# ZenHKD/ocr-vi-invoice

Hardware: AMD Instinct MI355X
Metric: invoice images/sec end-to-end (det+rec) (higher is better)
Workload: dtype f16x2

## Files before the change

include/ocrvi.h:

```cpp
#ifndef OCRVI_H
#define OCRVI_H

#include <stddef.h>
#include <stdint.h>

#ifdef __cplusplus
extern "C" {
#endif

#define OCRVI_OK 0
#define OCRVI_EINVAL (-1)
#define OCRVI_EHIP (-2)
#define OCRVI_ENOMEM (-3)
#define OCRVI_EBLOB (-4)
#define OCRVI_ERANGE (-5)

typedef enum { OCRVI_F32 = 0, OCRVI_BF16 = 1, OCRVI_F16 = 2, OCRVI_F16X2 = 3 } ocrvi_dtype;

const char* ocrvi_last_error(void);
int ocrvi_abi_version(void);

typedef struct ocrvi_det ocrvi_det;

typedef struct {
// ... 205 lines not shown
int ocrvi_edit_distance(int device, const int32_t* pred_ids, int T, const int32_t* pred_lens, const int32_t* gt_ids, int G,
                        const int32_t* gt_lens, int B, int32_t* dist, void* stream);

int ocrvi_test_offset_conv(int device, int dtype, const float* x, const float* weight_host, const float* bias_host, int N, int C, int H, int W,
                           int stride, float* out, int iters, float* avg_ms);
int ocrvi_test_deform_conv(int device, int dtype, const float* x, const float* offset, const float* mask,
                           const float* weight_host, const float* bias_host, int N, int C, int H, int W, int Co,
                           int stride, int relu, float* out, int iters, float* avg_ms);
int ocrvi_test_deform_conv_res(int device, int dtype, const float* x, const float* offset, const float* mask,
                               const float* weight_host, const float* bias_host, const float* res, int N, int C, int H, int W, int Co,
                               int stride, int relu, float* out, int iters, float* avg_ms);
int ocrvi_test_deform_conv_raw(int device, int dtype, const float* x, const float* offset, const float* mask,
                               const float* weight_host, const float* bias_host, const float* res, int N, int C, int H, int W, int Co,
                               int stride, int relu, void* out_raw, float* out);
int ocrvi_test_dcn_plan(int dtype, int N, int C, int H, int W, int Co, int stride, int n_cu, int32_t plan[8]);
int ocrvi_test_conv(int device, int dtype, const float* x, const float* weight_host, const float* bias_host,
                    int N, int C, int H, int W, int Co, int ksize, int sh, int sw, int groups, int act, float* out,
                    int iters, float* avg_ms);
int ocrvi_test_conv_res(int device, int dtype, const float* x, const float* weight_host, const float* bias_host, const float* res, int N,
                        int C, int H, int W, int Co, int ksize, int res_mode, int act, float* out, int iters, float* avg_ms);
int ocrvi_test_bneck_tail(int device, const float* t1, const float* identity, const float* w2_host, const float* b2_host,
                          const float* w3_host, const float* b3_host, const float* w1_host, const float* b1_host, int N, int H, int W,
                          int no_phase_c, float* y_out, float* t1n_out, int iters, float* avg_ms);
int ocrvi_test_db_tail(int device, int dtype, const float* x, const float* dc1_w_bin_host, const float* dc1_b_bin_host,
                       const float* dc1_w_thr_host, const float* dc1_b_thr_host, const float* dc2_w_bin_host, const float* dc2_b_bin_host,
                       const float* dc2_w_thr_host, const float* dc2_b_thr_host, int N, int OH, int OW, int groups, int binary_only,
                       float* out, float* out2, int iters, float* avg_ms);
int ocrvi_test_gemm(int device, int dtype, const float* a, const float* weight_host, const float* bias_host, const float* res, int M,
                    int K, int N, int act, int res_post, int out_f32, float* out, int iters, float* avg_ms);
int ocrvi_test_gemm_raw(int device, int dtype, const float* a, const float* weight_host, const float* bias_host, const float* res, int M,
                        int K, int N, int act, int res_post, int out_f32, void* out_raw, float* out);
int ocrvi_test_ring_plan(int dtype, int amode, int M, int K, int N, int out_f32, int has_res, int n_cu, int32_t plan[8]);
int ocrvi_test_conv_raw(int device, int dtype, const float* x, const float* weight_host, const float* bias_host, const float* res, int N,
                        int C, int H, int W, int Co, int ksize, int sh, int sw, int groups, int act, int res_post, int out_f32, int in_place,
                        void* out_raw, float* out);
int ocrvi_test_gconv_plan(int dtype, int N, int C, int H, int W, int Co, int sh, int sw, int groups, int out_f32, int has_res, int n_cu,
                          int32_t plan[12]);
int ocrvi_test_stem_pool(int device, int dtype, const float* x, const float* weight_host, const float* bias_host, int N, int H, int W, int fused,
                         float* out, int iters, float* avg_ms);
int ocrvi_test_attention(int device, int dtype, const float* qkv, int B, int N, int heads, float* out, int iters,
                         float* avg_ms);

int ocrvi_test_mlp(int device, int dtype, float* x, const float* ln_g_host, const float* ln_b_host, const float* w1_host, const float* b1_host,
                   const float* w2_host, const float* b2_host, const float* next_g_host, const float* next_b_host, int want_xn, int M, int D,
                   float* xn_out, int iters, float* avg_ms);
int ocrvi_test_mlp_raw(int device, int dtype, float* x, const float* ln_g_host, const float* ln_b_host, const float* w1_host, const float* b1_host,
// ... 23 lines not shown
```

ocr_vi_invoice_amd/_lib.py:

```python
from __future__ import annotations

import ctypes as C
import os
from typing import Optional

_HERE = os.path.dirname(os.path.abspath(__file__))
LIB_PATH = os.environ.get("OCRVI_LIB") or os.path.join(_HERE, "lib", "libocrvi.so")

OCRVI_F32, OCRVI_BF16, OCRVI_F16, OCRVI_F16X2 = 0, 1, 2, 3
DTYPES = {"f32": OCRVI_F32, "fp32": OCRVI_F32, "float32": OCRVI_F32, "bf16": OCRVI_BF16, "bfloat16": OCRVI_BF16,
          "f16": OCRVI_F16, "fp16": OCRVI_F16, "float16": OCRVI_F16,
          "f16x2": OCRVI_F16X2}
ABI_VERSION = 5

EXPORTS = [
    "ocrvi_last_error", "ocrvi_abi_version",
    "ocrvi_det_create", "ocrvi_det_destroy", "ocrvi_det_workspace_bytes", "ocrvi_det_forward", "ocrvi_det_debug_features",
    "ocrvi_rec_create", "ocrvi_rec_destroy", "ocrvi_rec_workspace_bytes", "ocrvi_rec_forward", "ocrvi_rec_debug_features",
    "ocrvi_ctc_greedy", "ocrvi_normalize_u8", "ocrvi_resize_u8", "ocrvi_crop_resize_normalize", "ocrvi_db_postprocess", "ocrvi_db_boxes_batch",
    "ocrvi_unclip_polygon", "ocrvi_db_components_workspace_bytes", "ocrvi_db_components", "ocrvi_db_boxes_batch_sparse",
    "ocrvi_test_deform_conv", "ocrvi_test_offset_conv", "ocrvi_test_conv", "ocrvi_test_gemm", "ocrvi_test_attention", "ocrvi_test_mlp", "ocrvi_test_stem_pool", "ocrvi_test_pack_f16x2",
    "ocrvi_prof_enable", "ocrvi_prof_reset", "ocrvi_prof_report",
    "ocrvi_det_status", "ocrvi_rec_status", "ocrvi_range_reset", "ocrvi_range_flag",
    "ocrvi_resize_normalize_pages", "ocrvi_crop_resize_normalize_pages", "ocrvi_db_boxes_pages",
    "ocrvi_det_binary_workspace_bytes", "ocrvi_det_forward_binary",
    "ocrvi_four_point_transform", "ocrvi_warp_perspective_u8", "ocrvi_warp_perspective_pages",
    "ocrvi_test_layernorm", "ocrvi_test_frm_vertical", "ocrvi_test_asf", "ocrvi_test_maxpool", "ocrvi_test_db_maps", "ocrvi_test_ctc_logsoftmax",
    "ocrvi_det_eval_workspace_bytes", "ocrvi_det_eval", "ocrvi_ctc_loss", "ocrvi_edit_distance",
    "ocrvi_test_deform_conv_res",
    "ocrvi_enhance_init", "ocrvi_enhance_tables", "ocrvi_enhance_workspace_bytes", "ocrvi_enhance_u8",
    "ocrvi_rgb_to_lab_u8", "ocrvi_lab_to_rgb_u8", "ocrvi_clahe_lab_u8", "ocrvi_nlm_lab_u8", "ocrvi_sharpen_u8",
    "ocrvi_min_area_quads", "ocrvi_quad_crops", "ocrvi_crop_quad_resize_normalize_pages", "ocrvi_crop_quad_resize_normalize",
    "ocrvi_jpeg_info", "ocrvi_jpeg_parse", "ocrvi_jpeg_table_entry", "ocrvi_jpeg_decode_pages",
    "ocrvi_test_conv_res", "ocrvi_test_db_tail",
    "ocrvi_db_target_jobs", "ocrvi_db_target_maps", "ocrvi_resize_normalize_pad_pages",
    "ocrvi_test_mlp_raw",
    "ocrvi_test_bneck_tail",
    "ocrvi_jpeg_quant_tables", "ocrvi_jpeg_encode_header", "ocrvi_jpeg_encode_sizes", "ocrvi_jpeg_encode_table_entry", "ocrvi_jpeg_encode_pages",
    "ocrvi_test_gemm_raw", "ocrvi_test_ring_plan",
    "ocrvi_overlay_segments", "ocrvi_overlay_pages",
    "ocrvi_test_deform_conv_raw", "ocrvi_test_dcn_plan",
    "ocrvi_test_conv_raw", "ocrvi_test_gconv_plan",
    "ocrvi_png_info", "ocrvi_png_parse", "ocrvi_png_table_entry", "ocrvi_png_plan", "ocrvi_png_decode_pages",
]
PAGE_ENTRY = 4
DET_EVAL_RECORD_BYTES = 104
DET_EVAL_INT_SLOTS = ("tp", "fp", "fn", "positive_count", "negatives", "negative_count")
DET_EVAL_F64_SLOTS = ("pos_bce", "topk_bce", "dice_inter", "pred_mask", "gt_mask", "l1_num", "thresh_mask")
CTC_LOSS_MAX_TARGET = 1024
EDIT_DISTANCE_MAX_LEN = 2048
CLAHE_WORKSPACE_BYTES = 16384
ENHANCE_MIN_SIDE = 16
DB_TARGET_GT, DB_TARGET_MASK, DB_TARGET_THRESH = 0, 1, 2
DB_TARGET_JOB = 8
DB_TARGET_MAX_SIDE = 16384
JPEG_ENTRY = 64
PNG_ENTRY = 16
JPEG_ENC_ENTRY = 64
JPEG_HEADER_MAX = 640
OVERLAY_SEG = 8
OVERLAY_PRIM = 8
OVERLAY_MAX_COORD = 16384


class DetCfg(C.Structure):
    _fields_ = [("dtype", C.c_int32), ("k", C.c_float), ("max_batch", C.c_int32), ("backbone", C.c_int32), ("no_dcn", C.c_int32),
# ... 59 lines not shown
    lib.ocrvi_db_components_workspace_bytes.restype = sz
    lib.ocrvi_db_components.argtypes = [i32, vp, i32, i32, i32, C.c_float, vp, vp, vp, i32, vp, vp, C.c_longlong, vp, vp]
    lib.ocrvi_db_boxes_batch_sparse.argtypes = [vp, vp, vp, i32, vp, vp, C.c_longlong, i32, i32, i32, C.c_float, i32, C.c_float, C.c_float,
                                                C.c_double, C.c_double, i32, i32, i32, vp, vp, i32, vp, i32, vp]
    lib.ocrvi_unclip_polygon.argtypes = [vp, i32, C.c_double, vp, i32, C.POINTER(i32)]
    lib.ocrvi_db_boxes_batch.argtypes = [vp, i32, i32, i32, C.c_float, C.c_float, i32, C.c_float, C.c_float, C.c_double, C.c_double, i32, i32, i32,
                                         vp, vp, i32, vp, i32]
    lib.ocrvi_resize_normalize_pages.argtypes = [i32, vp, i32, i32, i32, f32p, vp]
    lib.ocrvi_crop_resize_normalize_pages.argtypes = [i32, vp, i32, i32p, i32, i32, i32, f32p, vp]
    lib.ocrvi_four_point_transform.argtypes = [vp, vp, vp, i32p, i32p]
    lib.ocrvi_warp_perspective_u8.argtypes = [i32, vp, i32, i32, vp, vp, i32, i32, vp]
    lib.ocrvi_warp_perspective_pages.argtypes = [i32, vp, vp, vp, i32, vp]
    lib.ocrvi_db_boxes_pages.argtypes = [vp, i32, i32, i32, C.c_float, C.c_float, i32, C.c_float, C.c_float, vp, vp, vp, vp, vp,
                                         vp, i32, vp, vp, vp, i32, vp, vp, i32]
    lib.ocrvi_test_deform_conv.argtypes = [i32, i32, f32p, f32p, f32p, vp, vp, i32, i32, i32, i32, i32, i32, i32, f32p, i32,
                                           C.POINTER(C.c_float)]
    lib.ocrvi_test_deform_conv_res.argtypes = [i32, i32, f32p, f32p, f32p, vp, vp, f32p, i32, i32, i32, i32, i32, i32, i32, f32p, i32,
                                               C.POINTER(C.c_float)]
    lib.ocrvi_test_offset_conv.argtypes = [i32, i32, f32p, vp, vp, i32, i32, i32, i32, i32, f32p, i32, C.POINTER(C.c_float)]
    lib.ocrvi_test_conv.argtypes = [i32, i32, f32p, vp, vp, i32, i32, i32, i32, i32, i32, i32, i32, i32, i32, f32p, i32,
                                    C.POINTER(C.c_float)]
    lib.ocrvi_test_conv_res.argtypes = [i32, i32, f32p, vp, vp, f32p, i32, i32, i32, i32, i32, i32, i32, i32, f32p, i32, C.POINTER(C.c_float)]
    lib.ocrvi_test_bneck_tail.argtypes = [i32, f32p, f32p, vp, vp, vp, vp, vp, vp, i32, i32, i32, i32, f32p, f32p, i32, C.POINTER(C.c_float)]
    lib.ocrvi_test_db_tail.argtypes = [i32, i32, f32p, vp, vp, vp, vp, vp, vp, vp, vp, i32, i32, i32, i32, i32, f32p, f32p, i32,
                                       C.POINTER(C.c_float)]
    lib.ocrvi_test_gemm.argtypes = [i32, i32, f32p, vp, vp, f32p, i32, i32, i32, i32, i32, i32, f32p, i32, C.POINTER(C.c_float)]
    lib.ocrvi_test_gemm_raw.argtypes = [i32, i32, f32p, vp, vp, f32p, i32, i32, i32, i32, i32, i32, vp, f32p]
    lib.ocrvi_test_ring_plan.argtypes = [i32, i32, i32, i32, i32, i32, i32, i32, C.POINTER(C.c_int32)]
    lib.ocrvi_test_deform_conv_raw.argtypes = [i32, i32, f32p, f32p, f32p, vp, vp, f32p, i32, i32, i32, i32, i32, i32, i32, vp, f32p]
    lib.ocrvi_test_dcn_plan.argtypes = [i32, i32, i32, i32, i32, i32, i32, i32, C.POINTER(C.c_int32)]
    lib.ocrvi_test_conv_raw.argtypes = [i32, i32, f32p, vp, vp, f32p] + [i32] * 13 + [vp, f32p]
    lib.ocrvi_test_gconv_plan.argtypes = [i32] * 12 + [C.POINTER(C.c_int32)]
    lib.ocrvi_test_stem_pool.argtypes = [i32, i32, f32p, vp, vp, i32, i32, i32, i32, f32p, i32, C.POINTER(C.c_float)]
    lib.ocrvi_test_attention.argtypes = [i32, i32, f32p, i32, i32, i32, f32p, i32, C.POINTER(C.c_float)]
    lib.ocrvi_test_mlp.argtypes = [i32, i32, f32p, vp, vp, vp, vp, vp, vp, vp, vp, i32, i32, i32, f32p, i32, C.POINTER(C.c_float)]
    lib.ocrvi_test_mlp_raw.argtypes = [i32, i32, f32p, vp, vp, vp, vp, vp, vp, vp, vp, i32, i32, vp, f32p, i32, C.POINTER(C.c_float)]
    lib.ocrvi_test_pack_f16x2.argtypes = [f32p, sz, vp, C.POINTER(C.c_float)]
    lib.ocrvi_test_layernorm.argtypes = [i32, i32, f32p, i32, i32, vp, vp, i32, i32, f32p]
    lib.ocrvi_test_frm_vertical.argtypes = [i32, i32, f32p, vp, i32, i32, i32, i32, f32p]
    lib.ocrvi_test_asf.argtypes = [i32, i32, f32p, f32p, f32p, f32p, vp, vp, i32, i32, i32, f32p]
    lib.ocrvi_test_maxpool.argtypes = [i32, i32, f32p, i32, i32, i32, i32, f32p]
    lib.ocrvi_test_db_maps.argtypes = [i32, f32p, f32p, C.c_float, f32p, f32p, f32p, sz]
    lib.ocrvi_test_ctc_logsoftmax.argtypes = [i32, f32p, i32, i32, i32, i32, f32p, i32p]
    lib.ocrvi_det_eval_workspace_bytes.argtypes = [i32, i32, i32, C.POINTER(sz)]
    lib.ocrvi_det_eval.argtypes = [i32, f32p, f32p, f32p, f32p, f32p, f32p, f32p, f32p, i32, i32, i32, C.c_double, vp, vp, sz, vp]
    lib.ocrvi_ctc_loss.argtypes = [i32, f32p, i32, i32, i32, i32p, i32, i32p, i32p, i32, vp, vp]
    lib.ocrvi_edit_distance.argtypes = [i32, i32p, i32, i32p, i32p, i32, i32p, i32, i32p, vp]
# ... 85 lines not shown
```

ocr_vi_invoice_amd/csrc/det_model.hip:

```cpp
#include <algorithm>
#include <memory>

#include "model.h"

using namespace ocrvi;

namespace {
const int kBlocks50[4] = {3, 4, 6, 3}, kBlocks18[4] = {2, 2, 2, 2};
const int kWidth[4] = {64, 128, 256, 512};
struct ResBlock {
    ConvLayer conv1, conv2, off, conv3, down;
    bool dcn = false, has_down = false;
    int stride = 1;
    void* tail_w = nullptr;
    float* tail_bias = nullptr;
    float tail_ws3 = 1.f, tail_ws1 = 1.f;
    bool tail = false, tail_c = false;
};
}

struct ocrvi_det {
    int device = 0;
    ocrvi_det_cfg cfg{};
    DeviceStore store;
    ConvLayer stem;
    std::vector<ResBlock> layers[4];
    ConvLayer lat[4], fpn[4];
    float *asf_w = nullptr, *asf_b = nullptr;
    ConvLayer head_conv, head_dc1;
    float* dc2_wb = nullptr;
    Tensor tap_c[4], tap_fused;
    bool basic = false;
    int expansion = 4;
    RangeWatch range;
};

extern "C" int ocrvi_det_create(int device, const void* blob_p, size_t blob_bytes, const ocrvi_det_cfg* cfg, ocrvi_det** out) {
    OCRVI_CHECK(cfg && out, OCRVI_EINVAL, "det_create: null argument");
    OCRVI_CHECK(dtype_valid(cfg->dtype), OCRVI_EINVAL, "det_create: bad dtype %d", cfg->dtype);
    OCRVI_CHECK(cfg->backbone == 0 || cfg->backbone == 1, OCRVI_EINVAL, "det_create: backbone %d (0 = ResNet-50, 1 = ResNet-18)", cfg->backbone);
// ... 38 lines not shown
            if (bk.dcn) OCRVI_TRY(load_conv(st, blob, p + ".conv2.off", 27, w, 3, 1, AM_CONV3, dt, true, &bk.off));
            if (!basic) OCRVI_TRY(load_conv(st, blob, p + ".conv3", 4 * w, w, 1, 1, AM_CONV1, dt, true, &bk.conv3));
            if (bk.has_down) OCRVI_TRY(load_conv(st, blob, p + ".down", ex * w, inpl, 1, 1, AM_CONV1, dt, true, &bk.down));
            inpl = ex * w;
        }
        for (int b = 0; b < nblk && !basic && dt == OCRVI_F16X2; ++b) {
            ResBlock& bk = h->layers[li][b];
            if (bk.dcn || bk.stride != 1 || !bk.conv2.quartets || w != 64 || bk.conv2.Np != 64 || bk.conv2.Cin_g != 64) continue;
            const std::string p = "layer" + std::to_string(li + 1) + "." + std::to_string(b);
            const std::string pn = "layer" + std::to_string(li + 1) + "." + std::to_string(b + 1);
            const BlobTensor *w3 = nullptr, *b3 = nullptr, *w1 = nullptr, *b1 = nullptr;
            OCRVI_TRY(blob.get(p + ".conv3.w", 256, 64, 1, 1, &w3));
            OCRVI_TRY(blob.get(p + ".conv3.b", 256, 0, 0, 0, &b3));
            if (b + 1 < nblk) {
                OCRVI_TRY(blob.get(pn + ".conv1.w", 64, 256, 1, 1, &w1));
                OCRVI_TRY(blob.get(pn + ".conv1.b", 64, 0, 0, 0, &b1));
            }
            PackedBneckTail pt = pack_bneck_tail(w3->data, b3->data, w1 ? w1->data : nullptr, b1 ? b1->data : nullptr);
            OCRVI_TRY(st.upload(pt.stream.data(), pt.stream.size(), &bk.tail_w));
            OCRVI_TRY(st.upload_f32(pt.bias, &bk.tail_bias));
            bk.tail_ws3 = pt.ws3; bk.tail_ws1 = pt.ws1;
            bk.tail = true; bk.tail_c = w1 != nullptr;
        }
    }
    for (int i = 0; i < 4; ++i) {
        OCRVI_TRY(load_conv(st, blob, "neck.lat" + std::to_string(i), 256, ex * kWidth[i], 1, 1, AM_CONV1, dt, true, &h->lat[i]));
        OCRVI_TRY(load_conv(st, blob, "neck.fpn" + std::to_string(i), 256, 256, 3, 1, AM_CONV3, dt, true, &h->fpn[i], nullptr, true));
    }
    {
        const BlobTensor *w = nullptr, *b = nullptr;
        OCRVI_TRY(blob.get("neck.asf.w", 4, 1024, 0, 0, &w));
        OCRVI_TRY(blob.get("neck.asf.b", 4, 0, 0, 0, &b));
        OCRVI_TRY(st.upload(w->data, 4096 * 4, (void**)&h->asf_w));
        OCRVI_TRY(st.upload(b->data, 16, (void**)&h->asf_b));
    }
    OCRVI_TRY(load_conv(st, blob, "head.conv", 128, 256, 3, 1, AM_CONV3, dt, true, &h->head_conv, nullptr, true));
    {
        std::vector<float> w2(2 * 64 * 4), b2(2);
        const char* names[2] = {"head.bin", "head.thr"};
        const float *dw[2] = {nullptr, nullptr}, *db[2] = {nullptr, nullptr};
        for (int br = 0; br < 2; ++br) {
            const BlobTensor *w = nullptr, *b = nullptr, *ww = nullptr, *bb = nullptr;
            OCRVI_TRY(blob.get(std::string(names[br]) + ".dc1.w", 64, 64, 2, 2, &w));
            OCRVI_TRY(blob.get(std::string(names[br]) + ".dc1.b", 64, 0, 0, 0, &b));
            dw[br] = w->data;
            db[br] = b->data;
// ... 89 lines not shown
    Tensor idn;
    OCRVI_TRY(identity(r, bk, x, y, &idn));
    ConvOpts o = conv_opts(1, 1, ACT_RELU);
    o.res = &idn; o.res_mode = RES_SAME;
    if (bk.dcn) OCRVI_TRY(dcn_offsets(r, bk, t1, y.h, y.w, 1, &o.offs));
    return conv(r, bk.conv2, t1, y, o);
}

static int fused_bottleneck(Runner& r, const ResBlock& bk, const Tensor& x, const Tensor& y, const Tensor& t1, bool have_t1,
                            const Tensor& t1_next) {
    if (!have_t1) OCRVI_TRY(conv(r, bk.conv1, x, t1, conv_opts(1, 0, ACT_RELU)));
    Tensor idn;
    OCRVI_TRY(identity(r, bk, x, y, &idn));
    OCRVI_CHECK(idn.c == 256 && y.c == 256 && t1.c == 64 && !idn.f32 && !y.f32, OCRVI_EINVAL, "det: fused layer1 chain on a foreign shape");
    if (r.dry()) return OCRVI_OK;
    BneckTailParams q;
    q.x = t1.p; q.w2 = bk.conv2.w; q.wt = bk.tail_w; q.bias2 = bk.conv2.bias; q.bias_t = bk.tail_bias;
    q.idn = idn.p; q.y = y.p; q.t1n = bk.tail_c ? t1_next.p : nullptr;
    q.n_img = x.n; q.H = y.h; q.W = y.w;
    q.ws2 = bk.conv2.wscale; q.ws3 = bk.tail_ws3; q.ws1 = bk.tail_ws1;
    return launch_bneck_tail(q, r.stream);
}

static int det_layer(const ocrvi_det& h, Runner& r, int li, Tensor* x) {
    const std::vector<ResBlock>& blocks = h.layers[li];
    Tensor cur = *x;
    const int N = cur.n, w = kWidth[li], cw = h.expansion * w, nb = (int)blocks.size();
    const int lh = cur.h / blocks[0].stride, lw = cur.w / blocks[0].stride;
    Tensor tap = r.alloc(N, lh, lw, cw);
    const size_t slot_mark = r.arena.mark();
    Tensor slot[2] = {r.alloc(N, lh, lw, cw), r.alloc(N, lh, lw, cw)};
    const bool fused_layer = !h.basic && blocks[0].tail;
    Tensor t1pp[2];
    if (fused_layer) { t1pp[0] = r.alloc(N, lh, lw, w); t1pp[1] = r.alloc(N, lh, lw, w); }
    bool have_t1 = false;
    for (int b = 0; b < nb; ++b) {
        const ResBlock& bk = blocks[b];
        Tensor y = b == nb - 1 ? tap : slot[b & 1];
        const size_t block_mark = r.arena.mark();
        if (fused_layer && bk.tail) {
            OCRVI_TRY(fused_bottleneck(r, bk, cur, y, t1pp[b & 1], have_t1, t1pp[(b + 1) & 1]));
            have_t1 = bk.tail_c;
        } else if (h.basic) {
            OCRVI_TRY(basic_block(r, bk, cur, y, w));
        } else {
            OCRVI_TRY(bottleneck(r, bk, cur, y, w));
        }
        r.arena.release(block_mark);
        cur = y;
    }
    r.arena.release(slot_mark);
    *x = cur;
    return OCRVI_OK;
}

static int det_neck(const ocrvi_det& h, Runner& r, const Tensor* feats, Tensor* fused) {
    const int N = feats[0].n;
    Tensor inner[4], p[4];
    for (int i = 3; i >= 0; --i) {
        inner[i] = r.alloc(N, feats[i].h, feats[i].w, 256);
        ConvOpts o;
        if (i < 3) { o.res = &inner[i + 1]; o.res_mode = RES_UP2; }
        OCRVI_TRY(conv(r, h.lat[i], feats[i], inner[i], o));
        p[i] = r.alloc(N, feats[i].h, feats[i].w, 256);
        OCRVI_TRY(conv(r, h.fpn[i], inner[i], p[i], conv_opts(1, 1, ACT_RELU)));
// ... 101 lines not shown
```

ocr_vi_invoice_amd/csrc/kernels.h:

```cpp
#pragma once
#include "common.h"

namespace ocrvi {

int k_nchw3_to_nhwc4_pad(int dtype, const float* x, void* y, int N, int H, int W, int pad_t, int pad_l, int Hp, int Wp, hipStream_t s);
int k_maxpool3x3s2(int dtype, const void* x, void* y, int N, int H, int W, int C, hipStream_t s);
bool stem_pool_eligible(int dtype, int cout, int Kp, int KH, int H, int W);
int k_stem_pool(int dtype, const void* xpad, const void* w, const float* bias, float wscale, void* y, int N, int H, int W, int Hp, int Wp,
                hipStream_t s);
int k_layernorm(int dtype, const void* x, int x_f32, void* out, int out_f32, const float* gamma, const float* beta, int rows, int D,
                hipStream_t s);
bool mlp_fused_eligible(int dtype, int D);
bool mlp_x2_eligible(int dtype, int D);
void pack_mlp_x2_stream(const float* w1, const float* w2, int D, std::vector<char>& out);
int k_mlp_x2(float* x, void* xn, const float* ln_g, const float* ln_b, const float* next_g, const float* next_b, const void* wstream, const float* b1,
             const float* b2, int M, int D, hipStream_t s);
void pack_mlp_stream(const float* w1, const float* w2, int D, int dtype, std::vector<char>& out);
int k_mlp_fused(int dtype, float* x, void* xn, const float* ln_g, const float* ln_b, const float* next_g, const float* next_b, const void* wstream,
                const float* b1, const float* b2, int M, int D, hipStream_t s);
int k_cast_from_f32(int dtype, const float* x, void* y, size_t n, hipStream_t s);
int k_nhwc_to_nchw_f32(int dtype, const void* x, float* y, int N, int H, int W, int C, int ld, int coff, hipStream_t s);

int k_attention(int dtype, const void* qkv, void* out, int B, int N, int heads, hipStream_t s, void* scratch = nullptr);
size_t attention_scratch_bytes(int dtype, int B, int N, int heads);
int k_frm_vertical(int dtype, const void* kv, const float* vq, void* out, int B, int H, int W, int D, hipStream_t s);

int k_asf(int dtype, const void* p2, const void* p3, const void* p4, const void* p5, const float* w, const float* b, float* scratch, void* out,
          int N, int H, int W, hipStream_t s);
size_t asf_scratch_bytes(int N, int H, int W);
int k_db_maps(const float* bin_logits, const float* thresh_logits, float k, float* binary, float* thresh, float* thresh_binary, size_t n,
              hipStream_t s);

int k_ctc_logsoftmax_argmax(const float* logits, int ld, float* log_probs, int32_t* argmax_ids, int B, int T, int C, hipStream_t s);
int k_ctc_argmax_tbc(const float* log_probs, int32_t* argmax_ids, int B, int T, int C, hipStream_t s);
int k_ctc_collapse(const int32_t* argmax_ids, int32_t* ids, int32_t* lens, int B, int T, int blank, hipStream_t s);

}
```

ocr_vi_invoice_amd/csrc/mlp_x2.hip:

```cpp
#include <stdlib.h>
#include <string.h>

#include "gemm_ring.h"
#include "kernels.h"

namespace ocrvi {
OCRVI_RANGE_FLAG_TU()

struct MlpX2Params {
    float* x = nullptr;
    void* xn = nullptr;
    const float* ln_g = nullptr;
    const float* ln_b = nullptr;
    const float* next_g = nullptr;
    const float* next_b = nullptr;
    const char* wstream = nullptr;
    const float* b1 = nullptr;
    const float* b2 = nullptr;
    int M = 0;
};

template <int D, int R, int TB, bool SPLIT>
__global__ __launch_bounds__(512 / TB, TB == 2 ? 1 : 2) void mlp_x2_kernel(const MlpX2Params p) {
    typedef f16x2_t T;
    typedef Mma<T>::u4v U;
    constexpr int NWV = 8 / TB, NT = 64 * NWV;
    constexpr int KS = D / 32;
    constexpr int NCH = 4 * D / 32;
    constexpr int NB2 = D / 16;
    constexpr int W1B = 32 * D * 4;
    constexpr int UNIT = SPLIT ? W1B : 2 * W1B;
    constexpr int IPW = UNIT / 1024 / NWV;
    constexpr int PF = R - 1;
    constexpr int NU = (NCH + 1) * (SPLIT ? 2 : 1);
    static_assert(UNIT % (1024 * NWV) == 0 && R >= 2, "ring geometry");
    extern __shared__ __attribute__((aligned(16))) char smem[];
    const unsigned lds0 = (unsigned)(size_t)(__attribute__((address_space(3))) char*)smem;
    float* const c_b1 = (float*)(smem + R * UNIT);
    float* const c_b2 = c_b1 + 4 * D;
    float* const c_g = c_b2 + D;
    float* const c_be = c_g + D;
    float* const c_ng = c_be + D;
    float* const c_nb = c_ng + D;

    const int tid = threadIdx.x, lane = tid & 63;
    const int wave = __builtin_amdgcn_readfirstlane(tid >> 6);
    const int lr = lane & 15, g = lane >> 4;
    const bool next_ln = p.next_g != nullptr;
    for (int i = tid; i < 4 * D; i += NT) c_b1[i] = p.b1[i];
    for (int i = tid; i < D; i += NT) {
        c_b2[i] = p.b2[i];
        c_g[i] = p.ln_g[i];
        c_be[i] = p.ln_b[i];
        c_ng[i] = next_ln ? p.next_g[i] : 1.f;
        c_nb[i] = next_ln ? p.next_b[i] : 0.f;
    }
    const float* const tail = (const float*)(p.wstream + (size_t)(NCH + 1) * 2 * W1B);
    const float ws1 = tail[0], ws2 = tail[1];
    __syncthreads();

    const int ntiles = (p.M + 127) >> 7;
    const int G = gridDim.x;
    const int my_tiles = (ntiles - (int)blockIdx.x + G - 1) / G;

    const char* const wbase = uniform_ptr(p.wstream);
    int prod_slot = 0, prod_mod = 0, cons_slot = 0;
    auto issue_unit = [&]() {
        const char* src = wbase + (size_t)prod_mod * UNIT + wave * 1024;
        const unsigned dst = lds0 + prod_slot * UNIT + wave * 1024;
#pragma unroll
        for (int j = 0; j < IPW; ++j) glds16(src + j * (NWV * 1024), (unsigned)lane * 16u, __builtin_amdgcn_readfirstlane(dst + j * (NWV * 1024)));
        prod_slot = prod_slot + 1 == R ? 0 : prod_slot + 1;
        prod_mod = prod_mod + 1 == NU ? 0 : prod_mod + 1;
    };
    auto next_unit = [&]() -> const char* {
        wait_vm_barrier<(PF - 1) * IPW>();
        issue_unit();
        const char* s = smem + cons_slot * UNIT;
        cons_slot = cons_slot + 1 == R ? 0 : cons_slot + 1;
        return s;
    };
    for (int i = 0; i < PF; ++i) issue_unit();
    const int sw = swz128(lr);
    const int fo0 = ((2 * g) ^ sw) << 4, fo1 = ((2 * g + 1) ^ sw) << 4;
    unsigned long long range_mask = 0;

    for (int t = 0; t < my_tiles; ++t) {
        const int tile = (int)blockIdx.x + t * G;
        const int tok0 = tile * 128 + wave * (16 * TB);
        U xH[KS][TB], xL[KS][TB];
#pragma unroll
        for (int b = 0; b < TB; ++b) {
            float xv[KS][8];
            const int tok = min(tok0 + 16 * b + lr, p.M - 1);
            const float* xr = p.x + (size_t)tok * D + 8 * g;
#pragma unroll
            for (int ks = 0; ks < KS; ++ks) {
                const float4 v0 = *(const float4*)(xr + 32 * ks), v1 = *(const float4*)(xr + 32 * ks + 4);
                xv[ks][0] = v0.x; xv[ks][1] = v0.y; xv[ks][2] = v0.z; xv[ks][3] = v0.w;
                xv[ks][4] = v1.x; xv[ks][5] = v1.y; xv[ks][6] = v1.z; xv[ks][7] = v1.w;
            }
            float sum = 0.f;
#pragma unroll
            for (int ks = 0; ks < KS; ++ks)
#pragma unroll
                for (int e = 0; e < 8; ++e) sum += xv[ks][e];
            sum += __shfl_xor(sum, 16);
            sum += __shfl_xor(sum, 32);
            const float mean = sum / (float)D;
            float sq = 0.f;
#pragma unroll
            for (int ks = 0; ks < KS; ++ks)
#pragma unroll
                for (int e = 0; e < 8; ++e) { const float d = xv[ks][e] - mean; sq += d * d; }
            sq += __shfl_xor(sq, 16);
            sq += __shfl_xor(sq, 32);
            const float rstd = rsqrtf(sq / (float)D + 1e-5f);
#pragma unroll
            for (int ks = 0; ks < KS; ++ks) {
                float o[8];
#pragma unroll
                for (int q = 0; q < 2; ++q) {
                    const float4 gv = *(const float4*)(c_g + 32 * ks + 8 * g + 4 * q), bv = *(const float4*)(c_be + 32 * ks + 8 * g + 4 * q);
                    o[4 * q] = (xv[ks][4 * q] - mean) * rstd * gv.x + bv.x;
                    o[4 * q + 1] = (xv[ks][4 * q + 1] - mean) * rstd * gv.y + bv.y;
                    o[4 * q + 2] = (xv[ks][4 * q + 2] - mean) * rstd * gv.z + bv.z;
                    o[4 * q + 3] = (xv[ks][4 * q + 3] - mean) * rstd * gv.w + bv.w;
                }
                const uint4 c0 = Chunk<T>::pack(o), c1 = Chunk<T>::pack(o + 4);
                Mma<T>::regroup(c0, c1, xH[ks][b], xL[ks][b]);
            }
        }
        wait_vm_only<0>();

        f32x4 acc2[NB2][TB];
#pragma unroll
        for (int a = 0; a < NB2; ++a)
#pragma unroll
            for (int b = 0; b < TB; ++b) acc2[a][b] = (f32x4){0.f, 0.f, 0.f, 0.f};

        f32x4 hacc[2][TB], hprev[2][TB];
        constexpr int NV = 8 * TB;
        auto gelu_vals = [&](int i0, int i1, const float* bp) {
#pragma unroll
            for (int i = i0; i < i1; ++i) {
                const int b = i >> 3, a = (i >> 2) & 1, r = i & 3;
                hprev[a][b][r] = gelu_erf(hprev[a][b][r] * ws1 + bp[16 * a + r]);
            }
        };
        auto g1 = [&](const char* U1, bool with_gelu, const float* bv) {
#pragma unroll
            for (int a = 0; a < 2; ++a)
#pragma unroll
                for (int b = 0; b < TB; ++b) hacc[a][b] = (f32x4){0.f, 0.f, 0.f, 0.f};
            constexpr int P1 = TB == 2 ? 1 : 2;
            uint4 wr[P1 + 1][2][2];
            auto rd1 = [&](int ks, int set) {
#pragma unroll
                for (int a = 0; a < 2; ++a) {
                    const char* r = U1 + (ks * 32 + 16 * a + lr) * 128;
                    wr[set][a][0] = *(const uint4*)(r + fo0);
                    wr[set][a][1] = *(const uint4*)(r + fo1);
                }
            };
#pragma unroll
            for (int i = 0; i < P1; ++i) rd1(i, i);
            __builtin_amdgcn_sched_barrier(0);
#pragma unroll
            for (int ks = 0; ks < KS; ++ks) {
                if (ks + P1 < KS) rd1(ks + P1, (ks + P1) % (P1 + 1));
                __builtin_amdgcn_sched_barrier(0);
#pragma unroll
                for (int a = 0; a < 2; ++a)
#pragma unroll
                    for (int b = 0; b < TB; ++b)
                        Mma<T>::three(Mma<T>::as_u4v(wr[ks % (P1 + 1)][a][0]), Mma<T>::as_u4v(wr[ks % (P1 + 1)][a][1]), xH[ks][b], xL[ks][b], hacc[a][b]);
                if (with_gelu) gelu_vals(NV * ks / KS, NV * (ks + 1) / KS, bv);
                __builtin_amdgcn_sched_barrier(0);
            }
        };
        auto g2 = [&](const char* U2) {
            constexpr int GB = 2 / TB, NG = NB2 / GB, PFG = 2;
            uint4 w2r[PFG + 1][GB][2];
            auto rd2 = [&](int grp, int set) {
#pragma unroll
                for (int i = 0; i < GB; ++i) {
                    const char* r = U2 + (16 * (grp * GB + i) + lr) * 128;
                    w2r[set][i][0] = *(const uint4*)(r + fo0);
                    w2r[set][i][1] = *(const uint4*)(r + fo1);
                }
            };
#pragma unroll
            for (int i = 0; i < PFG; ++i) rd2(i, i);
            U hH[TB], hL[TB];
#pragma unroll
            for (int b = 0; b < TB; ++b) {
                const float h0[4] = {hprev[0][b][0], hprev[0][b][1], hprev[0][b][2], hprev[0][b][3]};
                const float h1[4] = {hprev[1][b][0], hprev[1][b][1], hprev[1][b][2], hprev[1][b][3]};
                range_mask |= f16x2_out_of_range(h0) | f16x2_out_of_range(h1);
                const uint4 c0 = Chunk<T>::pack(h0), c1 = Chunk<T>::pack(h1);
                Mma<T>::regroup(c0, c1, hH[b], hL[b]);
            }
            __builtin_amdgcn_sched_barrier(0);
#pragma unroll
            for (int grp = 0; grp < NG; ++grp) {
                if (grp + PFG < NG) rd2(grp + PFG, (grp + PFG) % (PFG + 1));
                __builtin_amdgcn_sched_barrier(0);
#pragma unroll
                for (int i = 0; i < GB; ++i)
#pragma unroll
                    for (int b = 0; b < TB; ++b)
                        Mma<T>::three(Mma<T>::as_u4v(w2r[grp % (PFG + 1)][i][0]), Mma<T>::as_u4v(w2r[grp % (PFG + 1)][i][1]), hH[b], hL[b], acc2[grp * GB + i][b]);
                __builtin_amdgcn_sched_barrier(0);
            }
        };
        auto keep = [&]() {
#pragma unroll
            for (int a = 0; a < 2; ++a)
#pragma unroll
                for (int b = 0; b < TB; ++b) hprev[a][b] = hacc[a][b];
        };
        auto second = [&](const char* U1) -> const char* {
            if constexpr (SPLIT) {
                return next_unit();
            } else {
                return U1 + W1B;
            }
        };
        auto bias_of = [&](int c) {
            int l = threadIdx.x;
            asm volatile("" : "+v"(l));
            return c_b1 + 32 * c + 4 * ((l & 63) >> 4);
        };
        {
            const char* const U1 = next_unit();
            g1(U1, false, bias_of(0));
            (void)second(U1);
        }
        keep();
        for (int k = 1; k < NCH; ++k) {
            const char* const U1 = next_unit();
            g1(U1, true, bias_of(k - 1));
            g2(second(U1));
            keep();
        }
        {
            const char* const U1 = next_unit();
            gelu_vals(0, NV, bias_of(NCH - 1));
            g2(second(U1));
        }

        const int pn_tok = lane >> 2, pn_g = lane & 3;
        const int pn_src = 4 * (16 * pn_g + pn_tok);
#pragma unroll
        for (int b = 0; b < TB; ++b) {
#pragma unroll
            for (int a = 0; a < NB2; ++a)
#pragma unroll
                for (int r = 0; r < 4; ++r)
                    acc2[a][b][r] = __int_as_float(__builtin_amdgcn_ds_bpermute(pn_src, __float_as_int(acc2[a][b][r])));
            const int tok = tok0 + 16 * b + pn_tok;
            const bool ok = tok < p.M;
            float* xr = p.x + (size_t)(ok ? tok : 0) * D + 4 * pn_g;
            float sum = 0.f;
            float4 rvs[NB2];
#pragma unroll
            for (int a = 0; a < NB2; ++a) rvs[a] = *(const float4*)(xr + 16 * a);
#pragma unroll
            for (int a = 0; a < NB2; ++a) {
                const float4 bv2 = *(const float4*)(c_b2 + 16 * a + 4 * pn_g);
                const float4 rv = rvs[a];
                f32x4 v = acc2[a][b];
                v[0] = v[0] * ws2 + bv2.x + rv.x; v[1] = v[1] * ws2 + bv2.y + rv.y; v[2] = v[2] * ws2 + bv2.z + rv.z; v[3] = v[3] * ws2 + bv2.w + rv.w;
                acc2[a][b] = v;
                if (ok) *(float4*)(xr + 16 * a) = make_float4(v[0], v[1], v[2], v[3]);
                sum += v[0] + v[1] + v[2] + v[3];
            }
            if (p.xn) {
                float mean = 0.f, rstd = 1.f;
                if (next_ln) {
                    sum += __shfl_xor(sum, 1);
                    sum += __shfl_xor(sum, 2);
                    mean = sum / (float)D;
                    float sq = 0.f;
#pragma unroll
// ... 57 lines not shown
            }
        }
    }
    std::vector<char> chunks(buf.size() * 4);
    convert_to_dtype(buf.data(), buf.size(), OCRVI_F16X2, chunks.data());
    out.assign(chunks.size() + 8, 0);
    for (size_t r = 0; r < nrows; ++r) {
        const uint64_t* src = (const uint64_t*)(chunks.data() + r * 128);
        uint64_t q[16];
        for (int k = 0; k < 4; ++k) {
            q[4 * k] = src[4 * k]; q[4 * k + 1] = src[4 * k + 2]; q[4 * k + 2] = src[4 * k + 1]; q[4 * k + 3] = src[4 * k + 3];
        }
        const int row = rowidx[r], sw = ((row >> 1) & 1) | (((row >> 3) & 1) << 2);
        uint64_t* dst = (uint64_t*)(out.data() + r * 128);
        for (int ch = 0; ch < 8; ++ch) {
            dst[2 * (ch ^ sw)] = q[2 * ch];
            dst[2 * (ch ^ sw) + 1] = q[2 * ch + 1];
        }
    }
    const float tail[2] = {1.0f / s1, 1.0f / s2};
    memcpy(out.data() + chunks.size(), tail, 8);
}

template <int D, int R, int TB, bool SPLIT>
static int launch_mlp_x2(const MlpX2Params& p, hipStream_t s) {
    const int smem = R * (SPLIT ? 128 : 256) * D + 9 * D * 4;
    auto kern = mlp_x2_kernel<D, R, TB, SPLIT>;
    OCRVI_TRY(ensure_max_smem((const void*)kern, smem));
    int n_cu = 0;
    OCRVI_TRY(device_cus(&n_cu));
    const int ntiles = (p.M + 127) / 128;
    int grid = std::min(ntiles, n_cu);
    grid = cdiv(ntiles, cdiv(ntiles, grid));
    hipLaunchKernelGGL(kern, dim3(grid), dim3(512 / TB), smem, s, p);
    OCRVI_HIP(hipGetLastError());
    return OCRVI_OK;
}

int k_mlp_x2(float* x, void* xn, const float* ln_g, const float* ln_b, const float* next_g, const float* next_b, const void* wstream, const float* b1,
             const float* b2, int M, int D, hipStream_t s) {
    OCRVI_CHECK((D == 128 || D == 256 || D == 384) && x && ln_g && ln_b && wstream && b1 && b2 && M > 0 && M < (1 << 24), OCRVI_EINVAL,
                "mlp_x2: bad argument (D %d, M %d)", D, M);
    MlpX2Params p;
    p.x = x; p.xn = xn; p.ln_g = ln_g; p.ln_b = ln_b; p.next_g = next_g; p.next_b = next_b; p.wstream = (const char*)wstream; p.b1 = b1; p.b2 = b2; p.M = M;
    char tag[64];
    snprintf(tag, sizeof(tag), "mlp_fused_d%d_f16x2", D);
    ProfScope ps(tag, 2.0 * M * 8.0 * D * D, (double)M * D * (8.0 + (xn ? 4.0 : 0.0)) + 8.0 * D * D * 4.0, s);
    if (D == 128) return launch_mlp_x2<128, 4, 1, false>(p, s);
    if (D == 256) return launch_mlp_x2<256, 2, 1, false>(p, s);
    return launch_mlp_x2<384, 3, 2, true>(p, s);
}

}
```

Baseline: 323.4.

## Fuse bottleneck conv3 and next block's conv1 into one chained MLP-style kernel

Adds a bottleneck mode to the fused two-GEMM MLP kernel so a block's conv3 (plus identity residual and ReLU) and the next block's conv1 (ReLU) run in one kernel. The conv3 output is written to y while staying in registers to feed conv1, which saves a kernel launch and a global re-read of the 4w-channel activation. It applies to detector layers of width 128/256 when the f16x2 path is eligible. The added identity prefetch and vmcnt-based pipelining make the kernel more complex and raise register pressure.

Result: no change. 326.3, median of 6 (+0.9%).

```diff
diff --git a/include/ocrvi.h b/include/ocrvi.h
--- a/include/ocrvi.h
+++ b/include/ocrvi.h
@@ -251,6 +251,9 @@
 int ocrvi_test_bneck_tail(int device, const float* t1, const float* identity, const float* w2_host, const float* b2_host,
                           const float* w3_host, const float* b3_host, const float* w1_host, const float* b1_host, int N, int H, int W,
                           int no_phase_c, float* y_out, float* t1n_out, int iters, float* avg_ms);
+int ocrvi_test_bneck_chain(int device, const float* t2, const float* identity, const float* w3_host, const float* b3_host,
+                           const float* w1_host, const float* b1_host, int N, int P, int H, int W, int idn_c, int idn_c0, float* y_out,
+                           float* t1n_out, int iters, float* avg_ms);
 int ocrvi_test_db_tail(int device, int dtype, const float* x, const float* dc1_w_bin_host, const float* dc1_b_bin_host,
                        const float* dc1_w_thr_host, const float* dc1_b_thr_host, const float* dc2_w_bin_host, const float* dc2_b_bin_host,
                        const float* dc2_w_thr_host, const float* dc2_b_thr_host, int N, int OH, int OW, int groups, int binary_only,
diff --git a/ocr_vi_invoice_amd/_lib.py b/ocr_vi_invoice_amd/_lib.py
--- a/ocr_vi_invoice_amd/_lib.py
+++ b/ocr_vi_invoice_amd/_lib.py
@@ -42,6 +42,7 @@
     "ocrvi_test_deform_conv_raw", "ocrvi_test_dcn_plan",
     "ocrvi_test_conv_raw", "ocrvi_test_gconv_plan",
     "ocrvi_png_info", "ocrvi_png_parse", "ocrvi_png_table_entry", "ocrvi_png_plan", "ocrvi_png_decode_pages",
+    "ocrvi_test_bneck_chain",
 ]
 PAGE_ENTRY = 4
 DET_EVAL_RECORD_BYTES = 104
@@ -147,7 +148,8 @@
                                     C.POINTER(C.c_float)]
     lib.ocrvi_test_conv_res.argtypes = [i32, i32, f32p, vp, vp, f32p, i32, i32, i32, i32, i32, i32, i32, i32, f32p, i32, C.POINTER(C.c_float)]
     lib.ocrvi_test_bneck_tail.argtypes = [i32, f32p, f32p, vp, vp, vp, vp, vp, vp, i32, i32, i32, i32, f32p, f32p, i32, C.POINTER(C.c_float)]
-    lib.ocrvi_test_db_tail.argtypes = [i32, i32, f32p, vp, vp, vp, vp, vp, vp, vp, vp, i32, i32, i32, i32, i32, f32p, f32p, i32,
+    lib.ocrvi_test_bneck_chain.argtypes = [i32, f32p, f32p, vp, vp, vp, vp, i32, i32, i32, i32, i32, i32, f32p, f32p, i32, C.POINTER(C.c_float)]
+    lib.ocrvi_test_db_tail.argtypes =[i32, i32, f32p, vp, vp, vp, vp, vp, vp, vp, vp, i32, i32, i32, i32, i32, f32p, f32p, i32,
                                        C.POINTER(C.c_float)]
     lib.ocrvi_test_gemm.argtypes = [i32, i32, f32p, vp, vp, f32p, i32, i32, i32, i32, i32, i32, f32p, i32, C.POINTER(C.c_float)]
     lib.ocrvi_test_gemm_raw.argtypes = [i32, i32, f32p, vp, vp, f32p, i32, i32, i32, i32, i32, i32, vp, f32p]
diff --git a/ocr_vi_invoice_amd/csrc/det_model.hip b/ocr_vi_invoice_amd/csrc/det_model.hip
--- a/ocr_vi_invoice_amd/csrc/det_model.hip
+++ b/ocr_vi_invoice_amd/csrc/det_model.hip
@@ -16,6 +16,9 @@
     float* tail_bias = nullptr;
     float tail_ws3 = 1.f, tail_ws1 = 1.f;
     bool tail = false, tail_c = false;
+    void* chain_w = nullptr;
+    float *chain_b3 = nullptr, *chain_b1 = nullptr;
+    bool chain = false;
 };
 }
 
@@ -100,6 +103,22 @@
             bk.tail_ws3 = pt.ws3; bk.tail_ws1 = pt.ws1;
             bk.tail = true; bk.tail_c = w1 != nullptr;
         }
+        for (int b = 0; b + 1 < nblk && !basic && (w == 128 || w == 256) && mlp_x2_eligible(dt, w); ++b) {
+            ResBlock& bk = h->layers[li][b];
+            const std::string p = "layer" + std::to_string(li + 1) + "." + std::to_string(b);
+            const std::string pn = "layer" + std::to_string(li + 1) + "." + std::to_string(b + 1);
+            const BlobTensor *w3 = nullptr, *b3 = nullptr, *w1 = nullptr, *b1 = nullptr;
+            OCRVI_TRY(blob.get(p + ".conv3.w", 4 * w, w, 1, 1, &w3));
+            OCRVI_TRY(blob.get(p + ".conv3.b", 4 * w, 0, 0, 0, &b3));
+            OCRVI_TRY(blob.get(pn + ".conv1.w", w, 4 * w, 1, 1, &w1));
+            OCRVI_TRY(blob.get(pn + ".conv1.b", w, 0, 0, 0, &b1));
+            std::vector<char> stream;
+            pack_mlp_x2_stream(w3->data, w1->data, w, stream);
+            OCRVI_TRY(st.upload(stream.data(), stream.size(), &bk.chain_w));
+            OCRVI_TRY(st.upload(b3->data, (size_t)4 * w * 4, (void**)&bk.chain_b3));
+            OCRVI_TRY(st.upload(b1->data, (size_t)w * 4, (void**)&bk.chain_b1));
+            bk.chain = true;
+        }
     }
     for (int i = 0; i < 4; ++i) {
         OCRVI_TRY(load_conv(st, blob, "neck.lat" + std::to_string(i), 256, ex * kWidth[i], 1, 1, AM_CONV1, dt, true, &h->lat[i]));
@@ -235,6 +254,24 @@
     return launch_bneck_tail(q, r.stream);
 }
 
+static int chain_bottleneck(Runner& r, const ResBlock& bk, const Tensor& x, const Tensor& y, int w, const Tensor& t1_own, bool have_t1,
+                            const Tensor& t1_next) {
+    Tensor t1 = t1_own;
+    if (!have_t1) {
+        t1 = r.alloc(x.n, x.h, x.w, w);
+        OCRVI_TRY(conv(r, bk.conv1, x, t1, conv_opts(1, 0, ACT_RELU)));
+    }
+    Tensor t2 = r.alloc(x.n, y.h, y.w, w);
+    ConvOpts o2 = conv_opts(bk.stride, 1, ACT_RELU);
+    if (bk.dcn) OCRVI_TRY(dcn_offsets(r, bk, t1, y.h, y.w, bk.stride, &o2.offs));
+    OCRVI_TRY(conv(r, bk.conv2, t1, t2, o2));
+    Tensor idn;
+    OCRVI_TRY(identity(r, bk, x, y, &idn));
+    OCRVI_CHECK(idn.c == 4 * w && y.c == 4 * w && t1_next.c == w && !idn.f32 && !y.f32, OCRVI_EINVAL, "det: fused conv3 -> conv1 chain on a foreign shape");
+    if (r.dry()) return OCRVI_OK;
+    return k_bneck_chain(t2.p, idn.p, idn.c, bk.chain_w, bk.chain_b3, bk.chain_b1, y.p, t1_next.p, y.n * y.h * y.w, w, r.stream);
+}
+
 static int det_layer(const ocrvi_det& h, Runner& r, int li, Tensor* x) {
     const std::vector<ResBlock>& blocks = h.layers[li];
     Tensor cur = *x;
@@ -243,9 +280,9 @@
     Tensor tap = r.alloc(N, lh, lw, cw);
     const size_t slot_mark = r.arena.mark();
     Tensor slot[2] = {r.alloc(N, lh, lw, cw), r.alloc(N, lh, lw, cw)};
-    const bool fused_layer = !h.basic && blocks[0].tail;
+    const bool fused_layer = !h.basic && blocks[0].tail, chain_layer = !h.basic && blocks[0].chain;
     Tensor t1pp[2];
-    if (fused_layer) { t1pp[0] = r.alloc(N, lh, lw, w); t1pp[1] = r.alloc(N, lh, lw, w); }
+    if (fused_layer || chain_layer) { t1pp[0] = r.alloc(N, lh, lw, w); t1pp[1] = r.alloc(N, lh, lw, w); }
     bool have_t1 = false;
     for (int b = 0; b < nb; ++b) {
         const ResBlock& bk = blocks[b];
@@ -254,6 +291,19 @@
         if (fused_layer && bk.tail) {
             OCRVI_TRY(fused_bottleneck(r, bk, cur, y, t1pp[b & 1], have_t1, t1pp[(b + 1) & 1]));
             have_t1 = bk.tail_c;
+        } else if (chain_layer && (bk.chain || have_t1)) {
+            if (bk.chain) {
+                OCRVI_TRY(chain_bottleneck(r, bk, cur, y, w, t1pp[b & 1], have_t1, t1pp[(b + 1) & 1]));
+            } else {
+                Tensor t2 = r.alloc(N, lh, lw, w);
+                ConvOpts o2 = conv_opts(bk.stride, 1, ACT_RELU);
+                if (bk.dcn) OCRVI_TRY(dcn_offsets(r, bk, t1pp[b & 1], lh, lw, bk.stride, &o2.offs));
+                OCRVI_TRY(conv(r, bk.conv2, t1pp[b & 1], t2, o2));
+                ConvOpts o3 = conv_opts(1, 0, ACT_RELU);
+                o3.res = &cur; o3.res_mode = RES_SAME;
+                OCRVI_TRY(conv(r, bk.conv3, t2, y, o3));
+            }
+            have_t1 = bk.chain;
         } else if (h.basic) {
             OCRVI_TRY(basic_block(r, bk, cur, y, w));
         } else {
diff --git a/ocr_vi_invoice_amd/csrc/kernels.h b/ocr_vi_invoice_amd/csrc/kernels.h
--- a/ocr_vi_invoice_amd/csrc/kernels.h
+++ b/ocr_vi_invoice_amd/csrc/kernels.h
@@ -15,6 +15,8 @@
 void pack_mlp_x2_stream(const float* w1, const float* w2, int D, std::vector<char>& out);
 int k_mlp_x2(float* x, void* xn, const float* ln_g, const float* ln_b, const float* next_g, const float* next_b, const void* wstream, const float* b1,
              const float* b2, int M, int D, hipStream_t s);
+int k_bneck_chain(const void* t2, const void* idn, int ldr, const void* wstream, const float* b3, const float* b1, void* y, void* t1n, int M, int P,
+                  hipStream_t s);
 void pack_mlp_stream(const float* w1, const float* w2, int D, int dtype, std::vector<char>& out);
 int k_mlp_fused(int dtype, float* x, void* xn, const float* ln_g, const float* ln_b, const float* next_g, const float* next_b, const void* wstream,
                 const float* b1, const float* b2, int M, int D, hipStream_t s);
diff --git a/ocr_vi_invoice_amd/csrc/mlp_x2.hip b/ocr_vi_invoice_amd/csrc/mlp_x2.hip
--- a/ocr_vi_invoice_amd/csrc/mlp_x2.hip
+++ b/ocr_vi_invoice_amd/csrc/mlp_x2.hip
@@ -18,10 +18,27 @@
     const float* b1 = nullptr;
     const float* b2 = nullptr;
     int M = 0;
+    const void* t2 = nullptr;
+    const void* idn = nullptr;
+    void* y = nullptr;
+    void* t1n = nullptr;
+    void* dump_page = nullptr;
+    int ldr = 0;
 };
 
-template <int D, int R, int TB, bool SPLIT>
+template <int OFF> __device__ __forceinline__ void gload16so(u32x4& dst, const char* sbase, unsigned voff) {
+    asm volatile("global_load_dwordx4 %0, %1, %2 offset:%3" : "=v"(dst) : "v"(voff), "s"(sbase), "n"(OFF) : "memory");
+}
+__device__ __forceinline__ float f16x2_elem(const u32x4& u, int r) {
+    union { unsigned w; f16_t h[2]; } c;
+    c.w = r < 2 ? u.x : u.y;
+    const unsigned lw = r < 2 ? u.z : u.w;
+    return (r & 1) ? fma_mix_hi(1.0f, lw, (float)c.h[1]) : fma_mix_lo(1.0f, lw, (float)c.h[0]);
+}
+
+template <int D, int R, int TB, bool SPLIT, bool BN = false>
 __global__ __launch_bounds__(512 / TB, TB == 2 ? 1 : 2) void mlp_x2_kernel(const MlpX2Params p) {
+    static_assert(!BN || (TB == 1 && !SPLIT), "bottleneck mode: 16 tokens per wave, whole stream units");
     typedef f16x2_t T;
     typedef Mma<T>::u4v U;
     constexpr int NWV = 8 / TB, NT = 64 * NWV;
@@ -50,10 +67,12 @@
     for (int i = tid; i < 4 * D; i += NT) c_b1[i] = p.b1[i];
     for (int i = tid; i < D; i += NT) {
         c_b2[i] = p.b2[i];
-        c_g[i] = p.ln_g[i];
-        c_be[i] = p.ln_b[i];
-        c_ng[i] = next_ln ? p.next_g[i] : 1.f;
-        c_nb[i] = next_ln ? p.next_b[i] : 0.f;
+        if constexpr (!BN) {
+            c_g[i] = p.ln_g[i];
+            c_be[i] = p.ln_b[i];
+            c_ng[i] = next_ln ? p.next_g[i] : 1.f;
+            c_nb[i] = next_ln ? p.next_b[i] : 0.f;
+        }
     }
     const float* const tail = (const float*)(p.wstream + (size_t)(NCH + 1) * 2 * W1B);
     const float ws1 = tail[0], ws2 = tail[1];
@@ -89,8 +108,24 @@
         const int tile = (int)blockIdx.x + t * G;
         const int tok0 = tile * 128 + wave * (16 * TB);
         U xH[KS][TB], xL[KS][TB];
-#pragma unroll
-        for (int b = 0; b < TB; ++b) {
+        u32x4 idr[2][2];
+        unsigned id_off = 0;
+        char* y_row = nullptr;
+        int y_step = 0;
+        const char* const id_base = uniform_ptr((const char*)p.idn);
+        if constexpr (BN) {
+            const int tok = tok0 + lr, tokc = min(tok, p.M - 1);
+            const uint4* tr = (const uint4*)((const char*)p.t2 + ((size_t)tokc * D + 8 * g) * 4);
+#pragma unroll
+            for (int ks = 0; ks < KS; ++ks) Mma<T>::regroup(tr[8 * ks], tr[8 * ks + 1], xH[ks][0], xL[ks][0]);
+#pragma unroll
+            for (int ks = 0; ks < KS; ++ks) asm volatile("" : "+v"(xH[ks][0]), "+v"(xL[ks][0]));
+            id_off = (unsigned)tokc * (unsigned)p.ldr * 4u + 16u * g;
+            y_row = tok < p.M ? (char*)p.y + ((size_t)tok * (4 * D) + 4 * g) * 4 : (char*)p.dump_page + lane * 16;
+            y_step = tok < p.M ? 128 : 0;
+        }
+#pragma unroll
+        for (int b = 0; b < (BN ? 0 : TB); ++b) {
             float xv[KS][8];
             const int tok = min(tok0 + 16 * b + lr, p.M - 1);
             const float* xr = p.x + (size_t)tok * D + 8 * g;
@@ -132,6 +167,10 @@
             }
         }
         wait_vm_only<0>();
+        if constexpr (BN) {
+            gload16so<0>(idr[0][0], id_base, id_off);
+            gload16so<64>(idr[0][1], id_base, id_off);
+        }
 
         f32x4 acc2[NB2][TB];
 #pragma unroll
@@ -148,7 +187,14 @@
                 hprev[a][b][r] = gelu_erf(hprev[a][b][r] * ws1 + bp[16 * a + r]);
             }
         };
-        auto g1 = [&](const char* U1, bool with_gelu, const float* bv) {
+        auto bn_vals = [&](int i0, int i1, const float* bp, int S) {
+#pragma unroll
+            for (int i = i0; i < i1; ++i) {
+                const int a = (i >> 2) & 1, r = i & 3;
+                hprev[a][0][r] = fmaxf(hprev[a][0][r] * ws1 + bp[16 * a + r] + f16x2_elem(idr[S][a], r), 0.f);
+            }
+        };
+        auto g1 = [&](const char* U1, bool with_gelu, const float* bv, int S = 0) {
 #pragma unroll
             for (int a = 0; a < 2; ++a)
 #pragma unroll
@@ -175,11 +221,15 @@
 #pragma unroll
                     for (int b = 0; b < TB; ++b)
                         Mma<T>::three(Mma<T>::as_u4v(wr[ks % (P1 + 1)][a][0]), Mma<T>::as_u4v(wr[ks % (P1 + 1)][a][1]), xH[ks][b], xL[ks][b], hacc[a][b]);
-                if (with_gelu) gelu_vals(NV * ks / KS, NV * (ks + 1) / KS, bv);
+                if constexpr (BN) {
+                    if (with_gelu) bn_vals(NV * ks / KS, NV * (ks + 1) / KS, bv, S);
+                } else {
+                    if (with_gelu) gelu_vals(NV * ks / KS, NV * (ks + 1) / KS, bv);
+                }
                 __builtin_amdgcn_sched_barrier(0);
             }
         };
-        auto g2 = [&](const char* U2) {
+        auto g2 = [&](const char* U2, int yc = 0, int S = -1) {
             constexpr int GB = 2 / TB, NG = NB2 / GB, PFG = 2;
             uint4 w2r[PFG + 1][GB][2];
             auto rd2 = [&](int grp, int set) {
@@ -200,8 +250,20 @@
                 range_mask |= f16x2_out_of_range(h0) | f16x2_out_of_range(h1);
                 const uint4 c0 = Chunk<T>::pack(h0), c1 = Chunk<T>::pack(h1);
                 Mma<T>::regroup(c0, c1, hH[b], hL[b]);
+                if constexpr (BN) {
+                    *(uint4*)(y_row + yc * y_step) = c0;
+                    *(uint4*)(y_row + yc * y_step + (y_step >> 1)) = c1;
+                }
             }
             __builtin_amdgcn_sched_barrier(0);
+            if constexpr (BN) {
+                if (S >= 0) {
+                    const unsigned o = id_off + (unsigned)(yc + 2) * 128u;
+                    gload16so<0>(idr[S][0], id_base, o);
+                    gload16so<64>(idr[S][1], id_base, o);
+                }
+                __builtin_amdgcn_sched_barrier(0);
+            }
 #pragma unroll
             for (int grp = 0; grp < NG; ++grp) {
                 if (grp + PFG < NG) rd2(grp + PFG, (grp + PFG) % (PFG + 1));
@@ -232,22 +294,64 @@
             asm volatile("" : "+v"(l));
             return c_b1 + 32 * c + 4 * ((l & 63) >> 4);
         };
-        {
-            const char* const U1 = next_unit();
-            g1(U1, false, bias_of(0));
-            (void)second(U1);
-        }
-        keep();
-        for (int k = 1; k < NCH; ++k) {
-            const char* const U1 = next_unit();
-            g1(U1, true, bias_of(k - 1));
-            g2(second(U1));
+        if constexpr (BN) {
+            constexpr int WA = (PF - 1) * IPW + 4 * PF, WB = 2 * IPW + 4;
+            static_assert(WA < 64 && WB < 64, "vmcnt is a 6-bit counter");
+            auto unit_bn = [&](bool lo) -> const char* {
+                if (lo) wait_vm_barrier<WA - 2>(); else wait_vm_barrier<WA>();
+                issue_unit();
+                const char* s = smem + cons_slot * UNIT;
+                cons_slot = cons_slot + 1 == R ? 0 : cons_slot + 1;
+                return s;
+            };
+            auto await_idn = [&](bool lo, int S) {
+                if (lo) wait_vm_only<WB - 2>(); else wait_vm_only<WB>();
+                bind16(idr[S][0]);
+                bind16(idr[S][1]);
+            };
+            auto step = [&](int k, int S, bool load) {
+                const char* const U1 = unit_bn(k <= PF);
+                await_idn(k == 1, S);
+                g1(U1, true, bias_of(k - 1), S);
+                g2(U1 + W1B, k - 1, load ? S : -1);
+                keep();
+            };
+            {
+                const char* const U1 = unit_bn(true);
+                g1(U1, false, bias_of(0));
+                gload16so<128>(idr[1][0], id_base, id_off);
+                gload16so<192>(idr[1][1], id_base, id_off);
+            }
             keep();
-        }
-        {
-            const char* const U1 = next_unit();
-            gelu_vals(0, NV, bias_of(NCH - 1));
-            g2(second(U1));
+            for (int k = 1; k < NCH - 1; k += 2) {
+                step(k, 0, true);
+                step(k + 1, 1, true);
+            }
+            step(NCH - 1, 0, false);
+            {
+                const char* const U1 = unit_bn(true);
+                await_idn(true, 1);
+                bn_vals(0, NV, bias_of(NCH - 1), 1);
+                g2(U1 + W1B, NCH - 1, -1);
+            }
+        } else {
+            {
+                const char* const U1 = next_unit();
+                g1(U1, false, bias_of(0));
+                (void)second(U1);
+            }
+            keep();
+            for (int k = 1; k < NCH; ++k) {
+                const char* const U1 = next_unit();
+                g1(U1, true, bias_of(k - 1));
+                g2(second(U1));
+                keep();
+            }
+            {
+                const char* const U1 = next_unit();
+                gelu_vals(0, NV, bias_of(NCH - 1));
+                g2(second(U1));
+            }
         }
 
         const int pn_tok = lane >> 2, pn_g = lane & 3;
@@ -261,6 +365,19 @@
                     acc2[a][b][r] = __int_as_float(__builtin_amdgcn_ds_bpermute(pn_src, __float_as_int(acc2[a][b][r])));
             const int tok = tok0 + 16 * b + pn_tok;
             const bool ok = tok < p.M;
+            if constexpr (BN) {
+                char* tr = ok ? (char*)p.t1n + ((size_t)tok * D + 4 * pn_g) * 4 : (char*)p.dump_page + lane * 16;
+#pragma unroll
+                for (int a = 0; a < NB2; ++a) {
+                    const float4 bv2 = *(const float4*)(c_b2 + 16 * a + 4 * pn_g);
+                    const f32x4 v = acc2[a][b];
+                    const float o[4] = {fmaxf(v[0] * ws2 + bv2.x, 0.f), fmaxf(v[1] * ws2 + bv2.y, 0.f), fmaxf(v[2] * ws2 + bv2.z, 0.f),
+                                        fmaxf(v[3] * ws2 + bv2.w, 0.f)};
+                    range_mask |= f16x2_out_of_range(o);
+                    *(uint4*)(tr + (ok ? 64 * a : 0)) = Chunk<T>::pack(o);
+                }
+                continue;
+            }
             float* xr = p.x + (size_t)(ok ? tok : 0) * D + 4 * pn_g;
             float sum = 0.f;
             float4 rvs[NB2];
@@ -364,10 +481,10 @@
     memcpy(out.data() + chunks.size(), tail, 8);
 }
 
-template <int D, int R, int TB, bool SPLIT>
+template <int D, int R, int TB, bool SPLIT, bool BN = false>
 static int launch_mlp_x2(const MlpX2Params& p, hipStream_t s) {
     const int smem = R * (SPLIT ? 128 : 256) * D + 9 * D * 4;
-    auto kern = mlp_x2_kernel<D, R, TB, SPLIT>;
+    auto kern = mlp_x2_kernel<D, R, TB, SPLIT, BN>;
     OCRVI_TRY(ensure_max_smem((const void*)kern, smem));
     int n_cu = 0;
     OCRVI_TRY(device_cus(&n_cu));
@@ -393,4 +510,23 @@
     return launch_mlp_x2<384, 3, 2, true>(p, s);
 }
 
-}
+int k_bneck_chain(const void* t2, const void* idn, int ldr, const void* wstream, const float* b3, const float* b1, void* y, void* t1n, int M, int P,
+                  hipStream_t s) {
+    OCRVI_CHECK((P == 128 || P == 256) && t2 && idn && wstream && b3 && b1 && y && t1n && M > 0 && M < (1 << 24), OCRVI_EINVAL,
+                "bneck_chain: bad argument (P %d, M %d)", P, M);
+    OCRVI_CHECK(ldr >= 4 * P && ldr % 4 == 0 && (size_t)M * ldr * 4 < ((size_t)1 << 32), OCRVI_EINVAL,
+                "bneck_chain: identity pitch %d (>= %d, a multiple of 4, M * pitch * 4 < 2^32)", ldr, 4 * P);
+    OCRVI_CHECK((((size_t)t2 | (size_t)idn | (size_t)y | (size_t)t1n | (size_t)wstream) & 15) == 0, OCRVI_EINVAL,
+                "bneck_chain: operands must be 16-byte aligned");
+    MlpX2Params p;
+    p.t2 = t2; p.idn = idn; p.ldr = ldr; p.wstream = (const char*)wstream; p.b1 = b3; p.b2 = b1; p.y = y; p.t1n = t1n; p.M = M;
+    const void* zero = nullptr;
+    OCRVI_TRY(ring_pages(&zero, &p.dump_page));
+    char tag[64];
+    snprintf(tag, sizeof(tag), "bneck_chain_d%d_f16x2", P);
+    ProfScope ps(tag, 2.0 * M * 8.0 * P * P, (double)M * P * 4.0 * 10.0 + 8.0 * P * P * 4.0, s);
+    if (P == 128) return launch_mlp_x2<128, 4, 1, false, true>(p, s);
+    return launch_mlp_x2<256, 2, 1, false, true>(p, s);
+}
+
+}
```
